# yewsiang/Transferable3D

Measured on AMD Instinct MI355X. Metric: frustums/sec fwd+bwd, higher is better.
Workload: dtype f32

## Files before the change

include/t3d.h:

```cpp
#ifndef T3D_H_
#define T3D_H_

#include <stdint.h>

#ifdef __cplusplus
extern "C" {
#endif

#define T3D_OK 0
#define T3D_ERR_ARG (-1)
#define T3D_ERR_SHAPE (-2)
#define T3D_ERR_LAUNCH (-3)
#define T3D_ERR_ABI (-4)

#define T3D_ABI_VERSION 3
#define T3D_V2_SIZE_pointmlp_fwd_args 200
#define T3D_V2_SIZE_pointmlp_dgrad_args 168
#define T3D_V2_SIZE_pointmlp_wgrad_args 144
#define T3D_V2_SIZE_pointmlp_dgrad_gram_args 168
#define T3D_V2_SIZE_pointmlp_gram_args 96
#define T3D_V2_SIZE_seg_head_args 208
#define T3D_V2_SIZE_boxpc_rep_args 104

#define T3D_TILE_ROWS 128
// ... 751 lines not shown
  const int32_t* choice;
  const int64_t* mask_offsets;
  uint64_t* masks;
  int32_t* seg_prefix;
  double* box2d_out;
  double* frustum_angle;
  int32_t* n_in_box;
  int32_t* count;
  int32_t* index;
  double* out_points;
  int32_t* label;
} t3d_frustum_extract_args;
#define T3D_V2_SIZE_frustum_extract_args 208
int t3d_frustum_extract(const t3d_frustum_extract_args* args, t3d_stream_t stream);

#ifdef __cplusplus
}
#endif
#endif
```

transferable3d_amd/abi.py:

```python
import ctypes as C
import os

F = C.POINTER(C.c_float)
I = C.POINTER(C.c_int32)
D = C.POINTER(C.c_double)
L = C.POINTER(C.c_int64)
i32, f32 = C.c_int, C.c_float

TILE_ROWS = 128
F32, BF16 = 0, 1
DTYPE_BY_NAME = {'f32': F32, 'bf16': BF16}
ARITH_AUTO, ARITH_FP32_MFMA, ARITH_BF16X3, ARITH_BF16 = 0, 1, 2, 3
ARITH_BY_NAME = {'auto': ARITH_AUTO, 'fp32_mfma': ARITH_FP32_MFMA, 'bf16x3': ARITH_BF16X3}
ARITH_NAMES = {ARITH_FP32_MFMA: 'fp32_mfma', ARITH_BF16X3: 'bf16x3', ARITH_BF16: 'bf16'}
ABI_VERSION = 3
ERR_ABI = -4
ACT_NONE, ACT_RELU, ACT_LEAKY_RELU, ACT_TANH = 0, 1, 2, 3
ACT_BY_NAME = {None: ACT_NONE, 'relu': ACT_RELU, 'leaky_relu': ACT_LEAKY_RELU, 'tanh': ACT_TANH}


class Sized(C.Structure):

    def __init__(self, *args, **kw):
        super().__init__(C.sizeof(type(self)), *args, **kw)
# ... 197 lines not shown
    _fields_ = [('off', C.c_int64), ('K', C.c_int32), ('N', C.c_int32), ('fwd', C.c_int32), ('dgrad', C.c_int32), ('blk0', C.c_int32), ('reserved', C.c_int32)]


def x3_frag_table(entries):
    import numpy as np
    rec = np.zeros(len(entries), dtype=np.dtype([('off', '<i8'), ('K', '<i4'), ('N', '<i4'), ('fwd', '<i4'), ('dgrad', '<i4'), ('blk0', '<i4'), ('reserved', '<i4')]))
    blk = 0
    for i, (off, K, N) in enumerate(entries):
        rec[i] = (off, K, N, 1, 1, blk, 0)
        blk += (K * N // 8 + 255) // 256
    return rec.view(np.uint8).copy(), blk


class SlabDesc(C.Structure):
    _fields_ = [('slab_off', C.c_int64), ('grad_off', C.c_int64), ('numel', C.c_int32), ('n_slabs', C.c_int32)]


class Schedule(C.Structure):
    _fields_ = [('base_lr', f32), ('lr_decay_rate', f32), ('lr_decay_step', f32), ('bn_init_decay', f32),
                ('bn_decay_rate', f32), ('bn_decay_step', f32), ('bn_decay_clip', f32), ('beta1', f32), ('beta2', f32),
                ('batch_size', i32), ('step_offset', i32)]


class BoxPcRepArgs(Sized):
    _fields_ = [('struct_size', C.c_uint32), ('pc', F), ('ld_pc', i32), ('C', i32), ('center', F), ('dims', F), ('theta', F), ('y_dims_cls', I),
                ('y_orient_cls', I), ('rep', F), ('ld_rep', i32), ('box_out', F), ('M', i32), ('rows_per_frustum', i32), ('rowmask', F)]


class BoxPcRepBArgs(C.Structure):
    _fields_ = [('center', F), ('dims', F), ('theta', F), ('y_dims_cls', I), ('y_orient_cls', I), ('box_out', F), ('pc', F), ('ld_pc', i32),
# ... 124 lines not shown
    't3d_boxpc_rep_b': [C.POINTER(BoxPcRepBArgs), VP],
    't3d_boxpc_rep_bwd': [C.POINTER(BoxPcRepBwdArgs), VP],
    't3d_boxpc_loss': [C.POINTER(BoxPcLossArgs), VP],
    't3d_pointmlp_dgrad_narrow': [C.POINTER(DgradNarrowArgs), VP],
    't3d_semi_final_loss': [C.POINTER(SemiFinalLossArgs), VP],
    't3d_anchor_reg_bwd': [C.POINTER(AnchorRegBwdArgs), VP],
    't3d_reduce_slabs': [F, F, C.POINTER(SlabDesc), i32, i32, VP],
    't3d_schedule_step': [F, C.POINTER(Schedule), VP],
    't3d_adam_tf_step': [F, F, F, F, C.c_int64, F, f32, f32, f32, f32, VP],
    't3d_momentum_step': [F, F, F, C.c_int64, F, f32, f32, VP],
    't3d_split_x3': [F, VP, C.c_int64, C.c_int64, VP],
    't3d_split_x3_frag': [F, VP, VP, C.c_int64, VP, i32, i32, VP],
    't3d_dropout_mask': [F, C.c_int64, f32, C.c_uint32, F, VP],
    't3d_cast_bf16': [F, VP, C.c_int64, VP],
    't3d_frustum_extract': [C.POINTER(FrustumExtractArgs), VP],
}

LIB_PATH = os.path.join(os.path.dirname(os.path.abspath(__file__)), 'libt3d.so')
ERRORS = {-1: 'T3D_ERR_ARG', -2: 'T3D_ERR_SHAPE', -3: 'T3D_ERR_LAUNCH'}


class T3DError(RuntimeError):
    pass


def source_hash_of(lib):
    buf = C.create_string_buffer(64)
    check(lib.t3d_source_hash(buf, 64), 't3d_source_hash')
    return buf.value.decode()

# ... 37 lines not shown
```

transferable3d_amd/csrc/bn_optim.hip:

```cpp
#include "common.h"
#include "poolbwd_dev.h"
#include "bn_dev.h"

namespace {

template <int GR, int CH = FC_CH>
__global__ __launch_bounds__(GR * CH) void k_bn_fwd_finalize(const t3d_bn_fwd_finalize_args p) {
  __shared__ double red[GR][CH];
  __shared__ float s_scsh[2 * CH];
  bn_fwd_finalize_body<GR, CH>(p, red, s_scsh, blockIdx.x);
}

__global__ __launch_bounds__(256) void k_pool_finalize(const t3d_pool_finalize_args p) {
  const int i = blockIdx.x * blockDim.x + threadIdx.x;
  if (i >= p.B * p.N) return;
  const int b = i / p.N, c = i % p.N;
  pool_pick_impl(p.pmax, p.pmin, p.pamax, p.pamin, p.tiles_per_frustum, p.N, b, c, p.scale[c], p.shift[c], p.pooled, p.ld_pooled,
                 p.argidx, p.ysel);
}

template <int GR, int CH = FC_CH>
__global__ __launch_bounds__(GR * CH) void k_bn_bwd_finalize(const t3d_bn_bwd_finalize_args p) {
  __shared__ double red[GR][CH];
  bn_bwd_finalize_body<GR, CH>(p, red, blockIdx.x, threadIdx.x);
// ... 53 lines not shown
    v[i] = vi;
    w[i] -= lr_t * mi / (sqrtf(vi) + eps);
  }
}

__global__ __launch_bounds__(256) void k_momentum_tf(float* __restrict__ w, const float* __restrict__ g, float* __restrict__ acc,
                                                     int64_t n, const float* __restrict__ hyper, float momentum, float gscale) {
  const float lr = hyper[1];
  for (int64_t i = (int64_t)blockIdx.x * blockDim.x + threadIdx.x; i < n; i += (int64_t)gridDim.x * blockDim.x) {
    const float a = fmaf(momentum, acc[i], g[i] * gscale);
    acc[i] = a;
    w[i] -= lr * a;
  }
}

__device__ __forceinline__ uint32_t mix_u32(uint64_t x) {
  x ^= x >> 33; x *= 0xff51afd7ed558ccdULL;
  x ^= x >> 33; x *= 0xc4ceb9fe1a85ec53ULL;
  x ^= x >> 33;
  return (uint32_t)(x >> 16);
}
__global__ __launch_bounds__(256) void k_dropout_mask(float* __restrict__ mask, int64_t n, float keep, uint32_t seed,
                                                      const float* __restrict__ hyper) {
  const uint64_t step = (uint64_t)hyper[0];
  const uint64_t key = ((uint64_t)seed << 32) ^ (step * 0x9E3779B97F4A7C15ULL);
  for (int64_t i = (int64_t)blockIdx.x * blockDim.x + threadIdx.x; i < n; i += (int64_t)gridDim.x * blockDim.x) {
    const uint32_t r = mix_u32(key + (uint64_t)i * 0xD6E8FEB86659FD93ULL);
    const float u = (float)(r >> 8) * (1.0f / 16777216.0f);
    mask[i] = u < keep ? 1.f : 0.f;
  }
// ... 87 lines not shown
  int64_t blocks = (n + 255) / 256;
  if (blocks > 2048) blocks = 2048;
  T3D_LAUNCH(k_adam_tf, dim3((unsigned)blocks), dim3(256), 0, static_cast<hipStream_t>(stream), params, grads, m,
                     v, n, hyper, beta1, beta2, eps, grad_scale);
  T3D_CHECK_LAUNCH();
  return T3D_OK;
}

extern "C" int t3d_momentum_step(float* params, const float* grads, float* accum, int64_t n, const float* hyper, float momentum,
                                 float grad_scale, t3d_stream_t stream) {
  if (!params || !grads || !accum || !hyper || n <= 0) return T3D_ERR_ARG;
  int64_t blocks = (n + 255) / 256;
  if (blocks > 2048) blocks = 2048;
  T3D_LAUNCH(k_momentum_tf, dim3((unsigned)blocks), dim3(256), 0, static_cast<hipStream_t>(stream), params, grads, accum, n, hyper,
             momentum, grad_scale);
  T3D_CHECK_LAUNCH();
  return T3D_OK;
}

__global__ __launch_bounds__(256) void k_cast_bf16(const float* __restrict__ src, bf16_t* __restrict__ dst, int64_t n) {
  const int64_t stride = (int64_t)gridDim.x * 256 * 8;
  for (int64_t i = ((int64_t)blockIdx.x * 256 + threadIdx.x) * 8; i < n; i += stride) {
    if (i + 8 <= n) {
      const float4 a = *reinterpret_cast<const float4*>(src + i), b = *reinterpret_cast<const float4*>(src + i + 4);
      const bf16x8 h = {(bf16_t)a.x, (bf16_t)a.y, (bf16_t)a.z, (bf16_t)a.w, (bf16_t)b.x, (bf16_t)b.y, (bf16_t)b.z, (bf16_t)b.w};
      *reinterpret_cast<bf16x8*>(dst + i) = h;
    } else {
      for (int64_t j = i; j < n; ++j) dst[j] = (bf16_t)src[j];
    }
  }
// ... 45 lines not shown
```

transferable3d_amd/csrc/common.h:

```cpp
#pragma once
#include <hip/hip_runtime.h>
#include <stdint.h>
#include "t3d.h"
#include "abi_take.h"

typedef float f32x16 __attribute__((ext_vector_type(16)));
typedef float f32x4 __attribute__((ext_vector_type(4)));

#define T3D_LAUNCH(...)          \
  do {                           \
    (void)hipGetLastError();     \
    hipLaunchKernelGGL(__VA_ARGS__); \
  } while (0)

#define T3D_CHECK_LAUNCH()                                  \
  do {                                                      \
    hipError_t e__ = hipGetLastError();                     \
    if (e__ != hipSuccess) return T3D_ERR_LAUNCH;           \
  } while (0)

__device__ __forceinline__ int xcd_remap(int bid, int nwg) {
  const int q = nwg >> 3, r = nwg & 7, xcd = bid & 7, idx = bid >> 3;
  const int base = (xcd < r) ? xcd * (q + 1) : r * (q + 1) + (xcd - r) * q;
  return base + idx;
// ... 39 lines not shown
  __device__ __forceinline__ static float ld1(const float* base, size_t i) { return (float)reinterpret_cast<const bf16_t*>(base)[i]; }
  __device__ __forceinline__ static void st1(float* base, size_t i, float v) { reinterpret_cast<bf16_t*>(base)[i] = (bf16_t)v; }
  __device__ __forceinline__ static void st2(float* base, size_t i, float a, float b) {
    bf16x2 v = {(bf16_t)a, (bf16_t)b};
    *reinterpret_cast<bf16x2*>(reinterpret_cast<bf16_t*>(base) + i) = v;
  }
  __device__ __forceinline__ static float rnd(float v) { return (float)(bf16_t)v; }
};

__device__ __forceinline__ float ld_elem(const float* base, size_t i, int dtype) {
  return dtype == T3D_BF16 ? Elem<bf16_t>::ld1(base, i) : base[i];
}
__device__ __forceinline__ float4 ld_elem4(const float* base, size_t i, int dtype) {
  return dtype == T3D_BF16 ? Elem<bf16_t>::widen(Elem<bf16_t>::ld4(base, i)) : *reinterpret_cast<const float4*>(base + i);
}
```

transferable3d_amd/csrc/pointmlp.hip:

```cpp
#include "common.h"
#include "poolbwd_dev.h"
#include "rider_dev.h"

#include <cstdlib>
#include <mutex>
#include <type_traits>
#include <utility>
#include <unordered_map>

namespace {

constexpr int BK = 32;
constexpr int MIN_WAVES_PER_EU = 2;
constexpr int LDR = BK + 4;
constexpr int NT = 256;

__device__ __forceinline__ float4 f4zero() { return make_float4(0.f, 0.f, 0.f, 0.f); }

__device__ __forceinline__ unsigned keep_bits32(const float* __restrict__ rowmask, int base) {
  float4 m[8];
#pragma unroll
  for (int q = 0; q < 8; ++q) m[q] = *reinterpret_cast<const float4*>(rowmask + base + (q >> 2) * 32 + (q & 3) * 8);
  unsigned bits = 0u;
#pragma unroll
// ... 665 lines not shown
    h_iter<1, TM, TN, SA, SB, LA, LB, AR, DIMA, BR, DIMB>(sa, sb, la, lb, smem, cur, last, last, a0, b0, acc, tid);
    cur ^= 1;
  }
  {
    const bf16_t* As = smem + cur * STAGE;
    const bf16_t* Bs = As + SA::LDS_ELEMS;
    mma_steps_h<TM, TN, AR, DIMA, BR, DIMB, 0, ST>(As, Bs, a0, b0, acc, tid & 63, [](int) {});
  }
  __syncthreads();
}

constexpr int BKX = 16;
constexpr int LDRX = BKX + 8;
constexpr int LDCX_PAD = 32;
__device__ __forceinline__ int x3_r_off(int row, int red) { return row * LDRX + red; }

__device__ __forceinline__ void split3(const float4& v, bf16x4& h, bf16x4& m, bf16x4& l) {
  const float x[4] = {v.x, v.y, v.z, v.w};
  unsigned hp[2], mp[2], lp[2];
  typedef float f32x2_ __attribute__((ext_vector_type(2)));
  auto pk = [](float a, float b) { const f32x2_ v = {a, b}; return __builtin_bit_cast(unsigned, __builtin_convertvector(v, bf16x2)); };
#pragma unroll
  for (int e = 0; e < 2; ++e) {
    const float x0 = x[2 * e], x1 = x[2 * e + 1];
    hp[e] = pk(x0, x1);
    float r0 = x0 - __uint_as_float(hp[e] << 16);
    asm("" : "+v"(r0));
    const float r1 = x1 - __uint_as_float(hp[e] & 0xffff0000u);
    mp[e] = pk(r0, r1);
    float s0 = r0 - __uint_as_float(mp[e] << 16);
    asm("" : "+v"(s0));
    const float s1 = r1 - __uint_as_float(mp[e] & 0xffff0000u);
    lp[e] = pk(s0, s1);
  }
  h = __builtin_bit_cast(bf16x4, make_uint2(hp[0], hp[1]));
  m = __builtin_bit_cast(bf16x4, make_uint2(mp[0], mp[1]));
  l = __builtin_bit_cast(bf16x4, make_uint2(lp[0], lp[1]));
}

struct WLoaderX3 {
  static constexpr bool PRESPLIT = true;
  const bf16_t* p;
  long stride;
  int ld;
  struct Raw { bf16x8 v; };
  struct Coef {};
  __device__ __forceinline__ Coef fetch_coef(int) const { return Coef(); }
  __device__ __forceinline__ Raw fetch(int plane, int row, int col) const {
    Raw r;
    r.v = *reinterpret_cast<const bf16x8*>(p + (size_t)plane * stride + (size_t)row * ld + col);
    return r;
  }
};
// ... 3725 lines not shown
```

transferable3d_amd/engine.py:

```python
import contextlib
import ctypes as C
import math
import os

import numpy as np
import torch

from . import abi
from .abi import fptr, iptr
from .constants import BN_EPS

TILE = abi.TILE_ROWS


class Runtime:

    def __init__(self, device=None, lib=None, gemm_arithmetic=None):
        self.lib = lib if lib is not None else abi.load()
        if gemm_arithmetic is None:
            gemm_arithmetic = 'fp32_mfma' if os.environ.get('T3D_X3', '1') == '0' else 'bf16x3'
        self.gemm_arithmetic = gemm_arithmetic
        self.arith = abi.ARITH_BY_NAME[gemm_arithmetic]
        if device is None:
            if not torch.cuda.is_available():
# ... 158 lines not shown
        n = int(np.prod(shape))
        n_pad = (n + 3) // 4 * 4
        if trainable:
            off = self.used
            assert off + n_pad <= self.params.numel(), 'VarStore capacity exceeded'
            self.used += n_pad
            buf = self.params
        else:
            off = self.state_used
            assert off + n_pad <= self.state.numel()
            self.state_used += n_pad
            buf = self.state
        self.index[name] = (off, tuple(shape), trainable)
        view = buf[off:off + n].view(*shape)
        view.copy_(torch.as_tensor(np.asarray(init, dtype=np.float32).reshape(shape)))
        return view

    def enable_bf16(self):
        if self.params16 is None:
            self.params16 = self.rt.zeros(self.params.numel(), dtype=torch.bfloat16)
        return self.params16

    def enable_x3(self):
        if getattr(self, 'params_x3', None) is None:
            self.params_x3 = self.rt.zeros(3 * self.params.numel(), dtype=torch.bfloat16)
        return self.params_x3

    def x3_ptr(self, w):
        off = (w.data_ptr() - self.params.data_ptr()) // 4
        if not (0 <= off and off + w.numel() <= self.params.numel() and w.is_contiguous()) or off % 4:
            return None, 0
        return self.enable_x3().data_ptr() + 2 * off, self.params.numel()

    def x3_frag(self, w, K, N):
        off = (w.data_ptr() - self.params.data_ptr()) // 4
        none = ((None, 0), (None, 0))
        if not (0 <= off and off + w.numel() <= self.params.numel() and w.is_contiguous()) or off % 8 or K % 32 or N % 32 or w.numel() != K * N:
            return none
        n = self.params.numel()
        stride = (n + 7) // 8 * 8
        if getattr(self, 'x3_frag_planes', None) is None:
            self.x3_frag_planes = (self.rt.zeros(3 * stride, dtype=torch.bfloat16), self.rt.zeros(3 * stride, dtype=torch.bfloat16))
            self.x3_frag_entries, self.x3_frag_stride, self.x3_frag_table = {}, stride, None
        self.x3_frag_entries[off] = (K, N)
        self.x3_frag_table = None
        pf, pd = self.x3_frag_planes
        return (pf.data_ptr() + 2 * off, stride), (pd.data_ptr() + 2 * off, stride)

    def frag_table(self):
        ent = getattr(self, 'x3_frag_entries', None)
        if not ent:
            return None
        if self.x3_frag_table is None:
            raw, blocks = abi.x3_frag_table([(off, K, N) for off, (K, N) in sorted(ent.items())])
            self.x3_frag_table = (torch.from_numpy(raw).to(self.rt.device), len(ent), blocks)
        return self.x3_frag_table

    def bf16_view(self, w):
        off = (w.data_ptr() - self.params.data_ptr()) // 4
        assert 0 <= off and off + w.numel() <= self.params.numel() and w.is_contiguous()
        return self.enable_bf16()[off:off + w.numel()].view(*w.shape)

    def get(self, name):
        off, shape, trainable = self.index[name]
        buf = self.params if trainable else self.state
        return buf[off:off + int(np.prod(shape))].view(*shape)

    def grad(self, name):
        off, shape, trainable = self.index[name]
        assert trainable
        return self.grads[off:off + int(np.prod(shape))].view(*shape)
# ... 11 lines not shown
        return self._alloc(name, shape, trainable, np.full(shape, val, np.float32))

    def state_dict(self):
        return {k: self.get(k).detach().cpu().numpy().copy() for k in self.index}

    def load_state_dict(self, sd, strict=True):
        for k, v in sd.items():
            if k not in self.index:
                if strict:
                    raise KeyError(k)
                continue
            v = np.asarray(v, dtype=np.float32)
            if v.size != int(np.prod(self.index[k][1])):
                raise ValueError('variable %s: the state holds shape %s, the graph declares %s' % (k, v.shape, self.index[k][1]))
            self.get(k).copy_(torch.as_tensor(v).reshape(self.index[k][1]))

    def trainable_ranges(self, prefixes=None):
        items = sorted((off, int(np.prod(shape)), name) for name, (off, shape, tr) in self.index.items() if tr)
        out = []
        for off, n, name in items:
            if prefixes is not None and not any(name.startswith(p) for p in prefixes):
                continue
            n_pad = (n + 3) // 4 * 4
            if out and out[-1][0] + out[-1][1] == off:
                out[-1][1] += n_pad
            else:
                out.append([off, n_pad])
        return [(o, n) for o, n in out]


# ... 542 lines not shown
```

transferable3d_amd/nets.py:

```python
import ctypes as C
import os

import numpy as np
import torch

from . import abi
from .abi import fptr, iptr
from .constants import BOX_OUT_DIMS, NUM_CLASS
from .engine import ActSpec, FcLayer, Plan, PointLayer, Runtime, VarStore, Workspace, TILE


class Graph:

    def __init__(self, batch_size, num_point, num_channel, rt=None, seed=0, unbiased_ema=True, vars=None, dtype='f32'):
        assert dtype in ('f32', 'bf16')
        self.dtype = dtype
        self.dt = abi.DTYPE_BY_NAME[dtype]
        self.adt = torch.bfloat16 if dtype == 'bf16' else torch.float32
        if num_point % TILE:
            raise abi.T3DError('num_point must be a multiple of %d' % TILE)
        self.rt = rt or Runtime()
        self.B, self.rpf, self.C = batch_size, num_point, num_channel
        self.ldpc = (num_channel + 3) // 4 * 4
        self.M = batch_size * num_point
# ... 25 lines not shown
        return self

    def emit_reduce_slabs(self, plan):
        ws, vs, lib = self.ws, self.vars, self.rt.lib
        plan.join()
        i0, i1 = self._slabs_reduced, len(ws.entries)
        self._slabs_reduced = i1
        if i1 == i0:
            return
        mx = max(e[2] for e in ws.entries[i0:i1])
        stride = C.sizeof(abi.SlabDesc)

        def thunk(s):
            return lib.t3d_reduce_slabs(fptr(ws.buf), fptr(vs.grads),
                                        C.cast(C.c_void_p(ws.table.data_ptr() + i0 * stride), C.POINTER(abi.SlabDesc)), i1 - i0, mx, s)
        plan.add_raw('t3d_reduce_slabs', thunk)

    def emit_cast_weights(self, plan):
        vs, lib = self.vars, self.rt.lib
        if self.dt != abi.BF16:
            from .engine import X3_PRESPLIT
            if (X3_PRESPLIT and self.rt.device.type == 'cuda' and self.rt.arith != abi.ARITH_FP32_MFMA and getattr(vs, 'x3_frag_enabled', True)
                    and hasattr(lib, 't3d_split_x3_frag')):
                def thunk(s):
                    if not getattr(vs, 'x3_frag_entries', None):
                        return 0
                    t, n, nblk = vs.frag_table()
                    pf, pd = vs.x3_frag_planes
                    return lib.t3d_split_x3_frag(fptr(vs.params), C.c_void_p(pf.data_ptr()), C.c_void_p(pd.data_ptr()), vs.x3_frag_stride,
                                                 C.c_void_p(t.data_ptr()), n, nblk, s)
                plan.add_raw('t3d_split_x3_frag', thunk)
            return
        p16 = vs.enable_bf16()
        plan.add_raw('t3d_cast_bf16', lambda s: lib.t3d_cast_bf16(fptr(vs.params), C.c_void_p(p16.data_ptr()), vs.used, s))

    def default_bucket(self):
        return self.vars.trainable_ranges(self.trained_prefixes)

    def declare_bucket(self, plan, prefixes):
        if not self.dp_buckets:
            return
        self.emit_reduce_slabs(plan)
        self.buckets.append(self.vars.trainable_ranges(prefixes))
        plan.bucket_ready(len(self.buckets) - 1)

# ... 22 lines not shown
        lib, hyper = self.rt.lib, self.hyper
        plan.add_raw('t3d_schedule_step', lambda s: lib.t3d_schedule_step(fptr(hyper), C.byref(sched), s), sched)

    def emit_dropout_masks(self, plan, seed=1234):
        lib, hyper = self.rt.lib, self.hyper
        for i, (scope, (mask, keep)) in enumerate(sorted(self.dropout_masks.items())):
            plan.add_raw('t3d_dropout_mask',
                         lambda s, mask=mask, keep=keep, sd=seed + 7919 * i: lib.t3d_dropout_mask(
                             fptr(mask), mask.numel(), keep, sd, fptr(hyper), s))

    def emit_adam(self, plan, prefixes=None, beta1=0.9, beta2=0.999, eps=1e-8, grad_scale=1.0):
        lib, vs, hyper = self.rt.lib, self.vars, self.hyper
        vs.optimizer_kind = 'adam'

        def adam(off, n):
            plan.add_raw('t3d_adam_tf_step',
                         lambda s, off=off, n=n: lib.t3d_adam_tf_step(
                             fptr(vs.params[off:]), fptr(vs.grads[off:]), fptr(vs.adam_m[off:]), fptr(vs.adam_v[off:]),
                             n, fptr(hyper), beta1, beta2, eps, grad_scale, s))
        self._emit_optimizer(plan, prefixes, adam)

    def emit_momentum(self, plan, prefixes=None, momentum=0.9, grad_scale=1.0):
        lib, vs, hyper = self.rt.lib, self.vars, self.hyper
        vs.optimizer_kind = 'momentum'

        def mom(off, n):
            plan.add_raw('t3d_momentum_step',
                         lambda s, off=off, n=n: lib.t3d_momentum_step(
                             fptr(vs.params[off:]), fptr(vs.grads[off:]), fptr(vs.adam_m[off:]), n, fptr(hyper), momentum, grad_scale, s))
        self._emit_optimizer(plan, prefixes, mom)

    def _emit_optimizer(self, plan, prefixes, launch):
        vs = self.vars
        self.trained_prefixes = prefixes
        ranges = vs.trainable_ranges(prefixes)
        if self.buckets:
            covered = sorted(r for b in self.buckets for r in b)
            assert sum(n for _, n in covered) == sum(n for _, n in ranges) and \
                all(any(o >= ro and o + n <= ro + rn for ro, rn in ranges) for o, n in covered), \
                'gradient buckets must partition the trained variables'
            for i, b in enumerate(self.buckets):
                plan.bucket_wait(i)
                for off, n in b:
                    launch(off, n)
# ... 971 lines not shown
```

transferable3d_amd/step.py:

```python
import os

import torch

from . import abi
from .engine import Plan


OPTIMIZER_CALLS = ('t3d_adam_tf_step', 't3d_momentum_step')


class TrainStep:
    def __init__(self, engine, pre, fwd, bwd=None, opt=None, process_group=None, use_hip_graph=None, force_dist=False,
                 one_graph=None):
        self.e, self.rt = engine, engine.rt
        self.pre, self.fwd, self.bwd, self.opt = pre, fwd, bwd, opt
        self.train = bwd is not None
        self.pg = process_group
        self.world = process_group.size() if process_group is not None else 1
        self.dist = self.train and process_group is not None and (self.world > 1 or force_dist)
        self.on_gpu = self.rt.device.type == 'cuda'
        want = use_hip_graph if use_hip_graph is not None else self.on_gpu
        self.want_graph = bool(want) and self.on_gpu
        env = os.environ.get('T3D_DP_ONE_GRAPH', '')
        if one_graph is None:
# ... 30 lines not shown
            for (name, call, arg), lane in zip(p.calls, p.lanes):
                if name == 't3d_dropout_mask' and not generate_masks:
                    continue
                calls.append((name, call, arg))
                lanes.append(lane)
            calls.append((Plan.JOIN, lambda s: 0, None))
            lanes.append(0)
            two = two or p.two_streams
        if self.dist and not any(c[0] == Plan.BUCKET for c in calls):
            k = next((i for i, c in enumerate(calls) if c[0] in OPTIMIZER_CALLS), len(calls))
            calls[k:k] = [(Plan.BUCKET, lambda s: 0, 0), (Plan.WAIT, lambda s: 0, 0)]
            lanes[k:k] = [0, 0]
        if not two:
            calls, lanes = self._overlap(calls, lanes)
            two = two or getattr(self, 'two_stream', False)
        prog, cur = [], Plan(self.rt)
        cur.two_streams = two

        def close():
            nonlocal cur
            if len(cur):
                prog.append(('run', cur))
            cur = Plan(self.rt)
            cur.two_streams = two

        for (name, call, arg), lane in zip(calls, lanes):
            if name in (Plan.BUCKET, Plan.WAIT):
                if self.dist:
                    close()
                    prog.append(('allreduce' if name == Plan.BUCKET else 'wait', arg))
# ... 32 lines not shown
        S_calls, T_calls = real(calls[sb:se]), real(calls[tb:sb])
        if self._two_stream_overlap(S_calls + T_calls):
            self.two_stream = True
            first, second = (T_calls, S_calls) if os.environ.get('T3D_TWO_STREAM_FIRST', 'S') == 'T' else (S_calls, T_calls)
            lanes2 = [0] * tb + [1] * len(first) + [0] + [0] * len(second) + [0]
            merged = first + [(Plan.FLUSH, lambda s: 0, None)] + second + [(Plan.JOIN, lambda s: 0, None)]
            calls = calls[:tb] + merged + calls[se + 1:]
            lanes2 += [0] * (len(calls) - len(lanes2))
            self.schedule_report = {'mode': 'two streams', 'S_launches': len(S_calls), 'T_launches': len(T_calls), 'hosted': 0, 'rider_ops': 0,
                                    'pairs': 0, 'solo': len(S_calls) + len(T_calls)}
            return calls, lanes2
        if self._sets is None:
            self._sets = schedule.RiderSets(self.rt)
        merged, self.schedule_report = schedule.overlap_chains(self.rt, S_calls, T_calls, self._sets)
        return calls[:tb] + merged + calls[se + 1:], lanes[:tb] + [0] * len(merged) + lanes[se + 1:]

    def _two_stream_overlap(self, chain_calls):
        mode = os.environ.get('T3D_OVERLAP_STREAMS', '')
        if mode in ('0', '1'):
            return mode == '1' and self.on_gpu
        if not self.on_gpu:
            return False
        return self.e.M >= 4 * 32768

    def _shares_gpu(self):
        if not self.on_gpu or os.environ.get('T3D_RIDERS_SHARED_GPU', '0') == '1':
            return False
        local_ranks = int(os.environ.get('LOCAL_WORLD_SIZE', self.world))
        return local_ranks > torch.cuda.device_count()

# ... 88 lines not shown
                graphs[k] = g
        return prog, graphs

    def run(self, generate_masks=True):
        self.n_runs += 1
        self._issue(generate_masks)
        if self._sets is not None and self.rider_check_every > 0 and self.n_runs % self.rider_check_every == 0:
            self.check_riders()

    def _issue(self, generate_masks):
        key = bool(generate_masks)
        ent = self.cache.get(key)
        if ent is None:
            ent = self.cache[key] = {'prog': self._program(key), 'graphs': None, 'runs': 0}
        ent['runs'] += 1
        if not self.want_graph or ent['runs'] == 1:
            return self._run_program(ent['prog'])
        if ent['graphs'] is None:
            prog, graphs = self._capture(ent['prog'])
            ent['cprog'], ent['graphs'] = prog, graphs
            if self._sets is not None:
                self._sets.timeouts()
        if ent['cprog'] and ent['cprog'][0][0] == 'run_graph':
            ent['graphs'][0].replay()
            return
        self._run_program(ent['cprog'], ent['graphs'])

    def dp_report(self):
        mode = 'flat' if len(self._buckets()) == 1 else 'bucketed'
        if self.one_graph:
# ... 211 lines not shown
```

Measured before the change: 27290.

## Fuse slab reduction, optimizer update and x3 weight split into one kernel

Adds a fused optimizer kernel driven by a per-block descriptor table. In one launch it sums gradient slabs, applies the Adam or momentum update, and writes the bf16x3 split weight planes for fragment tiles. The step program drops the separate reduce_slabs and split_x3_frag launches, which removes extra passes over params and grads and a few kernel launches per step. The cost is tracking when the planes are valid on the host, a tile layout that writes the planes from small 8x32 tiles, and a fallback to the old path whenever the setup does not fit the fused layout.

```diff
diff --git a/include/t3d.h b/include/t3d.h
--- a/include/t3d.h
+++ b/include/t3d.h
@@ -789,6 +789,39 @@
 #define T3D_V2_SIZE_frustum_extract_args 208
 int t3d_frustum_extract(const t3d_frustum_extract_args* args, t3d_stream_t stream);
 
+enum { T3D_OPT_FLAT = 0, T3D_OPT_SLAB = 1, T3D_OPT_TILE = 2 };
+enum { T3D_OPT_ADAM = 0, T3D_OPT_MOMENTUM = 1 };
+typedef struct {
+  int32_t kind;
+  int32_t count;
+  int64_t start;
+  int64_t slab_off;
+  int32_t n_slabs;
+  int32_t numel;
+  int64_t off;
+  int32_t K, N;
+  int32_t k0, n0;
+  int32_t fwd, dgrad;
+} t3d_opt_block;
+typedef struct {
+  uint32_t struct_size;
+  int32_t kind;
+  float* params;
+  float* grads;
+  float* m;
+  float* v;
+  const float* slab_base;
+  void* planes_fwd;
+  void* planes_dgrad;
+  int64_t plane_stride;
+  const t3d_opt_block* blocks;
+  int32_t n_blocks;
+  const float* hyper;
+  float beta1, beta2, eps, momentum, grad_scale;
+} t3d_optimizer_fused_args;
+#define T3D_V2_SIZE_optimizer_fused_args 120
+int t3d_optimizer_fused(const t3d_optimizer_fused_args* args, t3d_stream_t stream);
+
 #ifdef __cplusplus
 }
 #endif
diff --git a/transferable3d_amd/abi.py b/transferable3d_amd/abi.py
--- a/transferable3d_amd/abi.py
+++ b/transferable3d_amd/abi.py
@@ -235,6 +235,55 @@
 
 class SlabDesc(C.Structure):
     _fields_ = [('slab_off', C.c_int64), ('grad_off', C.c_int64), ('numel', C.c_int32), ('n_slabs', C.c_int32)]
+
+
+OPT_FLAT, OPT_SLAB, OPT_TILE = 0, 1, 2
+OPT_ADAM, OPT_MOMENTUM = 0, 1
+OPT_FLAT_ELEMS, OPT_SLAB_ELEMS = 1024, 256
+
+
+class OptimizerFusedArgs(Sized):
+    _fields_ = [('struct_size', C.c_uint32), ('kind', C.c_int32), ('params', C.c_void_p), ('grads', C.c_void_p), ('m', C.c_void_p), ('v', C.c_void_p),
+                ('slab_base', C.c_void_p), ('planes_fwd', C.c_void_p), ('planes_dgrad', C.c_void_p), ('plane_stride', C.c_int64),
+                ('blocks', C.c_void_p), ('n_blocks', C.c_int32), ('hyper', C.c_void_p), ('beta1', C.c_float), ('beta2', C.c_float),
+                ('eps', C.c_float), ('momentum', C.c_float), ('grad_scale', C.c_float)]
+
+
+def optimizer_fused_blocks(off, n, slabs, frags):
+    import numpy as np
+    dt = np.dtype([('kind', '<i4'), ('count', '<i4'), ('start', '<i8'), ('slab_off', '<i8'), ('n_slabs', '<i4'), ('numel', '<i4'), ('off', '<i8'),
+                   ('K', '<i4'), ('N', '<i4'), ('k0', '<i4'), ('n0', '<i4'), ('fwd', '<i4'), ('dgrad', '<i4')])
+    assert dt.itemsize == 64
+    end = off + n
+    by_off = {}
+    for so, go, ne, ns in slabs:
+        if go < off or go + ne > end or ne <= 0 or ns <= 0 or go in by_off:
+            return None
+        by_off[go] = (so, ne, ns)
+    recs, covered = [], []
+    for fo, K, N, fwd, dgrad in frags:
+        if fo < off or fo + K * N > end or fo % 8 or K % 32 or N % 32:
+            return None
+        so, ne, ns = by_off.pop(fo, (0, K * N, 0))
+        if ne != K * N or so % 4:
+            return None
+        covered.append((fo, K * N))
+        for k0 in range(0, K, 8):
+            for n0 in range(0, N, 32):
+                recs.append((OPT_TILE, 0, 0, so, ns, ne, fo, K, N, k0, n0, int(bool(fwd)), int(bool(dgrad))))
+    for go, (so, ne, ns) in sorted(by_off.items()):
+        covered.append((go, ne))
+        for s0 in range(0, ne, OPT_SLAB_ELEMS):
+            recs.append((OPT_SLAB, min(OPT_SLAB_ELEMS, ne - s0), go + s0, so, ns, ne, go, 0, 0, 0, 0, 0, 0))
+    pos = off
+    for co, cn in sorted(covered) + [(end, 0)]:
+        if co < pos:
+            return None
+        for s0 in range(pos, co, OPT_FLAT_ELEMS):
+            recs.append((OPT_FLAT, min(OPT_FLAT_ELEMS, co - s0), s0, 0, 0, 0, 0, 0, 0, 0, 0, 0, 0))
+        pos = co + cn
+    recs.sort(key=lambda r: -(r[4] if r[0] != OPT_FLAT else 0))
+    return np.array(recs, dtype=dt)
 
 
 class Schedule(C.Structure):
@@ -389,6 +438,7 @@
     't3d_dropout_mask': [F, C.c_int64, f32, C.c_uint32, F, VP],
     't3d_cast_bf16': [F, VP, C.c_int64, VP],
     't3d_frustum_extract': [C.POINTER(FrustumExtractArgs), VP],
+    't3d_optimizer_fused': [C.POINTER(OptimizerFusedArgs), VP],
 }
 
 LIB_PATH = os.path.join(os.path.dirname(os.path.abspath(__file__)), 'libt3d.so')
diff --git a/transferable3d_amd/csrc/bn_optim.hip b/transferable3d_amd/csrc/bn_optim.hip
--- a/transferable3d_amd/csrc/bn_optim.hip
+++ b/transferable3d_amd/csrc/bn_optim.hip
@@ -91,6 +91,170 @@
   }
 }
 
+__device__ __forceinline__ float opt_elem(const t3d_optimizer_fused_args& p, const bool adam, const float lr_t, const float lr, const float w,
+                                          const float g, float& m, float& v) {
+#pragma clang fp contract(off)
+  if (adam) {
+    const float gi = g * p.grad_scale;
+    const float mi = p.beta1 * m + (1.f - p.beta1) * gi;
+    const float vi = p.beta2 * v + (1.f - p.beta2) * gi * gi;
+    m = mi;
+    v = vi;
+    return w - lr_t * mi / (sqrtf(vi) + p.eps);
+  }
+  const float a = fmaf(p.momentum, m, g * p.grad_scale);
+  m = a;
+  return fmaf(-lr, a, w);
+}
+
+__device__ __forceinline__ float4 opt_elem4(const t3d_optimizer_fused_args& p, const bool adam, const float lr_t, const float lr, const float4 w,
+                                            const float4 g, float4& m, float4& v) {
+  float4 r;
+  r.x = opt_elem(p, adam, lr_t, lr, w.x, g.x, m.x, v.x);
+  r.y = opt_elem(p, adam, lr_t, lr, w.y, g.y, m.y, v.y);
+  r.z = opt_elem(p, adam, lr_t, lr, w.z, g.z, m.z, v.z);
+  r.w = opt_elem(p, adam, lr_t, lr, w.w, g.w, m.w, v.w);
+  return r;
+}
+
+__device__ __forceinline__ float4 slab_group_sum(const float4* __restrict__ s, const size_t n4, const int n_slabs, const int grp) {
+  float4 a0 = make_float4(0.f, 0.f, 0.f, 0.f), a1 = a0, a2 = a0, a3 = a0;
+  int k = grp;
+  for (; k + 56 < n_slabs; k += 64) {
+    float4 v[8];
+#pragma unroll
+    for (int u = 0; u < 8; ++u) v[u] = s[(size_t)(k + 8 * u) * n4];
+#pragma unroll
+    for (int u = 0; u < 8; u += 4) {
+      a0.x += v[u].x; a0.y += v[u].y; a0.z += v[u].z; a0.w += v[u].w;
+      a1.x += v[u + 1].x; a1.y += v[u + 1].y; a1.z += v[u + 1].z; a1.w += v[u + 1].w;
+      a2.x += v[u + 2].x; a2.y += v[u + 2].y; a2.z += v[u + 2].z; a2.w += v[u + 2].w;
+      a3.x += v[u + 3].x; a3.y += v[u + 3].y; a3.z += v[u + 3].z; a3.w += v[u + 3].w;
+    }
+  }
+  for (; k + 24 < n_slabs; k += 32) {
+    const float4 v0 = s[(size_t)(k + 0) * n4], v1 = s[(size_t)(k + 8) * n4], v2 = s[(size_t)(k + 16) * n4], v3 = s[(size_t)(k + 24) * n4];
+    a0.x += v0.x; a0.y += v0.y; a0.z += v0.z; a0.w += v0.w;
+    a1.x += v1.x; a1.y += v1.y; a1.z += v1.z; a1.w += v1.w;
+    a2.x += v2.x; a2.y += v2.y; a2.z += v2.z; a2.w += v2.w;
+    a3.x += v3.x; a3.y += v3.y; a3.z += v3.z; a3.w += v3.w;
+  }
+  for (; k < n_slabs; k += 8) {
+    const float4 v = s[(size_t)k * n4];
+    a0.x += v.x; a0.y += v.y; a0.z += v.z; a0.w += v.w;
+  }
+  float4 r;
+  r.x = (a0.x + a1.x) + (a2.x + a3.x); r.y = (a0.y + a1.y) + (a2.y + a3.y);
+  r.z = (a0.z + a1.z) + (a2.z + a3.z); r.w = (a0.w + a1.w) + (a2.w + a3.w);
+  return r;
+}
+
+constexpr int OPT_FLAT_ELEMS = 1024;
+constexpr int OPT_SLAB_ELEMS = 256;
+
+__global__ __launch_bounds__(512) void k_optimizer_fused(const t3d_optimizer_fused_args p) {
+  __shared__ float4 part[8][64];
+  __shared__ float wt[8][33];
+  const t3d_opt_block bl = p.blocks[blockIdx.x];
+  const int tid = threadIdx.x;
+  const bool adam = p.kind == T3D_OPT_ADAM;
+  const float lr_t = p.hyper[3], lr = p.hyper[1];
+  float4 zero = make_float4(0.f, 0.f, 0.f, 0.f);
+  if (bl.kind == T3D_OPT_FLAT) {
+    const int rem = bl.count - 4 * tid;
+    if (tid >= OPT_FLAT_ELEMS / 4 || rem <= 0) return;
+    const int64_t i = bl.start + 4 * tid;
+    if (rem >= 4 && (i & 3) == 0) {
+      float4 m = *reinterpret_cast<const float4*>(p.m + i), v = adam ? *reinterpret_cast<const float4*>(p.v + i) : zero;
+      const float4 w = opt_elem4(p, adam, lr_t, lr, *reinterpret_cast<const float4*>(p.params + i), *reinterpret_cast<const float4*>(p.grads + i), m, v);
+      *reinterpret_cast<float4*>(p.m + i) = m;
+      if (adam) *reinterpret_cast<float4*>(p.v + i) = v;
+      *reinterpret_cast<float4*>(p.params + i) = w;
+    } else {
+      for (int64_t j = i; j < i + (rem < 4 ? rem : 4); ++j) {
+        float m = p.m[j], v = adam ? p.v[j] : 0.f;
+        p.params[j] = opt_elem(p, adam, lr_t, lr, p.params[j], p.grads[j], m, v);
+        p.m[j] = m;
+        if (adam) p.v[j] = v;
+      }
+    }
+    return;
+  }
+  const bool tile = bl.kind == T3D_OPT_TILE;
+  if (!tile && ((bl.slab_off | bl.off | (int64_t)bl.numel) & 3) != 0) {
+    if (tid >= bl.count) return;
+    const int64_t e = bl.start - bl.off + tid, j = bl.start + tid;
+    float acc = 0.f;
+    for (int k = 0; k < bl.n_slabs; ++k) acc += p.slab_base[bl.slab_off + (size_t)k * bl.numel + e];
+    p.grads[j] = acc;
+    float m = p.m[j], v = adam ? p.v[j] : 0.f;
+    p.params[j] = opt_elem(p, adam, lr_t, lr, p.params[j], acc, m, v);
+    p.m[j] = m;
+    if (adam) p.v[j] = v;
+    return;
+  }
+  const int el = tid & 63, grp = tid >> 6;
+  const size_t n4 = (size_t)(bl.numel >> 2);
+  const size_t e4 = tile ? (((size_t)(bl.k0 + (el >> 3)) * bl.N + bl.n0) >> 2) + (el & 7) : (size_t)((bl.start - bl.off) >> 2) + el;
+  const bool live = el < (tile ? 64 : (bl.count >> 2));
+  const bool upd = grp == 0 && live;
+  const size_t ue = (size_t)(bl.off >> 2) + e4;
+  float4 w4 = zero, m4 = zero, v4 = zero, g4 = zero;
+  if (upd) {
+    w4 = reinterpret_cast<const float4*>(p.params)[ue];
+    m4 = reinterpret_cast<const float4*>(p.m)[ue];
+    if (adam) v4 = reinterpret_cast<const float4*>(p.v)[ue];
+    if (bl.n_slabs <= 0) g4 = reinterpret_cast<const float4*>(p.grads)[ue];
+  }
+  if (bl.n_slabs > 0) {
+    part[grp][el] = live ? slab_group_sum(reinterpret_cast<const float4*>(p.slab_base + bl.slab_off) + e4, n4, bl.n_slabs, grp) : zero;
+    __syncthreads();
+    if (upd) {
+      g4 = part[0][el];
+#pragma unroll
+      for (int g = 1; g < 8; ++g) {
+        const float4 u = part[g][el];
+        g4.x += u.x; g4.y += u.y; g4.z += u.z; g4.w += u.w;
+      }
+      reinterpret_cast<float4*>(p.grads)[ue] = g4;
+    }
+  }
+  if (upd) {
+    w4 = opt_elem4(p, adam, lr_t, lr, w4, g4, m4, v4);
+    reinterpret_cast<float4*>(p.m)[ue] = m4;
+    if (adam) reinterpret_cast<float4*>(p.v)[ue] = v4;
+    reinterpret_cast<float4*>(p.params)[ue] = w4;
+    if (tile) {
+      float* d = &wt[tid >> 3][(tid & 7) * 4];
+      d[0] = w4.x; d[1] = w4.y; d[2] = w4.z; d[3] = w4.w;
+    }
+  }
+  if (!tile) return;
+  __syncthreads();
+  bf16x4 h0, m0, l0, h1, m1, l1;
+  if (tid < 32 && bl.fwd) {
+    const int NB = bl.N / 32;
+    const long f = ((long)(bl.k0 >> 4) * NB + (bl.n0 >> 5)) * 64 + (((bl.k0 >> 3) & 1) << 5) + tid;
+    split3(make_float4(wt[0][tid], wt[1][tid], wt[2][tid], wt[3][tid]), h0, m0, l0);
+    split3(make_float4(wt[4][tid], wt[5][tid], wt[6][tid], wt[7][tid]), h1, m1, l1);
+    bf16_t* d = static_cast<bf16_t*>(p.planes_fwd) + bl.off + f * 8;
+    *reinterpret_cast<bf16x8*>(d) = __builtin_shufflevector(h0, h1, 0, 1, 2, 3, 4, 5, 6, 7);
+    *reinterpret_cast<bf16x8*>(d + p.plane_stride) = __builtin_shufflevector(m0, m1, 0, 1, 2, 3, 4, 5, 6, 7);
+    *reinterpret_cast<bf16x8*>(d + 2 * p.plane_stride) = __builtin_shufflevector(l0, l1, 0, 1, 2, 3, 4, 5, 6, 7);
+  }
+  if (tid >= 64 && tid < 96 && bl.dgrad) {
+    const int t = tid - 64, r = t >> 2, k = bl.k0 + r, nn = bl.n0 + 8 * (t & 3), KB = bl.K / 32;
+    const long f = ((long)(nn >> 4) * KB + (k >> 5)) * 64 + (((nn >> 3) & 1) << 5) + (k & 31);
+    const float* src = &wt[r][8 * (t & 3)];
+    split3(make_float4(src[0], src[1], src[2], src[3]), h0, m0, l0);
+    split3(make_float4(src[4], src[5], src[6], src[7]), h1, m1, l1);
+    bf16_t* d = static_cast<bf16_t*>(p.planes_dgrad) + bl.off + f * 8;
+    *reinterpret_cast<bf16x8*>(d) = __builtin_shufflevector(h0, h1, 0, 1, 2, 3, 4, 5, 6, 7);
+    *reinterpret_cast<bf16x8*>(d + p.plane_stride) = __builtin_shufflevector(m0, m1, 0, 1, 2, 3, 4, 5, 6, 7);
+    *reinterpret_cast<bf16x8*>(d + 2 * p.plane_stride) = __builtin_shufflevector(l0, l1, 0, 1, 2, 3, 4, 5, 6, 7);
+  }
+}
+
 __device__ __forceinline__ uint32_t mix_u32(uint64_t x) {
   x ^= x >> 33; x *= 0xff51afd7ed558ccdULL;
   x ^= x >> 33; x *= 0xc4ceb9fe1a85ec53ULL;
@@ -208,6 +372,23 @@
   if (blocks > 2048) blocks = 2048;
   T3D_LAUNCH(k_momentum_tf, dim3((unsigned)blocks), dim3(256), 0, static_cast<hipStream_t>(stream), params, grads, accum, n, hyper,
              momentum, grad_scale);
+  T3D_CHECK_LAUNCH();
+  return T3D_OK;
+}
+
+static_assert(sizeof(t3d_optimizer_fused_args) == T3D_V2_SIZE_optimizer_fused_args && sizeof(t3d_opt_block) == 64, "t3d.h: t3d_optimizer_fused");
+
+extern "C" int t3d_optimizer_fused(const t3d_optimizer_fused_args* a, t3d_stream_t stream) {
+  T3D_ABI_TAKE(optimizer_fused_args, a);
+  if (!a || !a->params || !a->grads || !a->m || !a->hyper || !a->blocks || a->n_blocks <= 0) return T3D_ERR_ARG;
+  if (a->kind != T3D_OPT_ADAM && a->kind != T3D_OPT_MOMENTUM) return T3D_ERR_ARG;
+  if (a->kind == T3D_OPT_ADAM && !a->v) return T3D_ERR_ARG;
+  auto misaligned = [](const void* q) { return (reinterpret_cast<uintptr_t>(q) & 15) != 0; };
+  if (misaligned(a->params) || misaligned(a->grads) || misaligned(a->m) || misaligned(a->v) || misaligned(a->slab_base) ||
+      misaligned(a->planes_fwd) || misaligned(a->planes_dgrad) || (reinterpret_cast<uintptr_t>(a->blocks) & 7))
+    return T3D_ERR_ARG;
+  if ((a->planes_fwd || a->planes_dgrad) && (a->plane_stride <= 0 || (a->plane_stride & 7))) return T3D_ERR_ARG;
+  T3D_LAUNCH(k_optimizer_fused, dim3((unsigned)a->n_blocks), dim3(512), 0, static_cast<hipStream_t>(stream), *a);
   T3D_CHECK_LAUNCH();
   return T3D_OK;
 }
diff --git a/transferable3d_amd/csrc/common.h b/transferable3d_amd/csrc/common.h
--- a/transferable3d_amd/csrc/common.h
+++ b/transferable3d_amd/csrc/common.h
@@ -77,3 +77,26 @@
 __device__ __forceinline__ float4 ld_elem4(const float* base, size_t i, int dtype) {
   return dtype == T3D_BF16 ? Elem<bf16_t>::widen(Elem<bf16_t>::ld4(base, i)) : *reinterpret_cast<const float4*>(base + i);
 }
+
+__device__ __forceinline__ void split3(const float4& v, bf16x4& h, bf16x4& m, bf16x4& l) {
+  const float x[4] = {v.x, v.y, v.z, v.w};
+  unsigned hp[2], mp[2], lp[2];
+  typedef float f32x2_ __attribute__((ext_vector_type(2)));
+  auto pk = [](float a, float b) { const f32x2_ v = {a, b}; return __builtin_bit_cast(unsigned, __builtin_convertvector(v, bf16x2)); };
+#pragma unroll
+  for (int e = 0; e < 2; ++e) {
+    const float x0 = x[2 * e], x1 = x[2 * e + 1];
+    hp[e] = pk(x0, x1);
+    float r0 = x0 - __uint_as_float(hp[e] << 16);
+    asm("" : "+v"(r0));
+    const float r1 = x1 - __uint_as_float(hp[e] & 0xffff0000u);
+    mp[e] = pk(r0, r1);
+    float s0 = r0 - __uint_as_float(mp[e] << 16);
+    asm("" : "+v"(s0));
+    const float s1 = r1 - __uint_as_float(mp[e] & 0xffff0000u);
+    lp[e] = pk(s0, s1);
+  }
+  h = __builtin_bit_cast(bf16x4, make_uint2(hp[0], hp[1]));
+  m = __builtin_bit_cast(bf16x4, make_uint2(mp[0], mp[1]));
+  l = __builtin_bit_cast(bf16x4, make_uint2(lp[0], lp[1]));
+}
diff --git a/transferable3d_amd/csrc/pointmlp.hip b/transferable3d_amd/csrc/pointmlp.hip
--- a/transferable3d_amd/csrc/pointmlp.hip
+++ b/transferable3d_amd/csrc/pointmlp.hip
@@ -703,29 +703,6 @@
 constexpr int LDRX = BKX + 8;
 constexpr int LDCX_PAD = 32;
 __device__ __forceinline__ int x3_r_off(int row, int red) { return row * LDRX + red; }
-
-__device__ __forceinline__ void split3(const float4& v, bf16x4& h, bf16x4& m, bf16x4& l) {
-  const float x[4] = {v.x, v.y, v.z, v.w};
-  unsigned hp[2], mp[2], lp[2];
-  typedef float f32x2_ __attribute__((ext_vector_type(2)));
-  auto pk = [](float a, float b) { const f32x2_ v = {a, b}; return __builtin_bit_cast(unsigned, __builtin_convertvector(v, bf16x2)); };
-#pragma unroll
-  for (int e = 0; e < 2; ++e) {
-    const float x0 = x[2 * e], x1 = x[2 * e + 1];
-    hp[e] = pk(x0, x1);
-    float r0 = x0 - __uint_as_float(hp[e] << 16);
-    asm("" : "+v"(r0));
-    const float r1 = x1 - __uint_as_float(hp[e] & 0xffff0000u);
-    mp[e] = pk(r0, r1);
-    float s0 = r0 - __uint_as_float(mp[e] << 16);
-    asm("" : "+v"(s0));
-    const float s1 = r1 - __uint_as_float(mp[e] & 0xffff0000u);
-    lp[e] = pk(s0, s1);
-  }
-  h = __builtin_bit_cast(bf16x4, make_uint2(hp[0], hp[1]));
-  m = __builtin_bit_cast(bf16x4, make_uint2(mp[0], mp[1]));
-  l = __builtin_bit_cast(bf16x4, make_uint2(lp[0], lp[1]));
-}
 
 struct WLoaderX3 {
   static constexpr bool PRESPLIT = true;
diff --git a/transferable3d_amd/engine.py b/transferable3d_amd/engine.py
--- a/transferable3d_amd/engine.py
+++ b/transferable3d_amd/engine.py
@@ -196,6 +196,8 @@
         self.index[name] = (off, tuple(shape), trainable)
         view = buf[off:off + n].view(*shape)
         view.copy_(torch.as_tensor(np.asarray(init, dtype=np.float32).reshape(shape)))
+        if trainable:
+            self.invalidate_planes()
         return view
 
     def enable_bf16(self):
@@ -224,8 +226,11 @@
         if getattr(self, 'x3_frag_planes', None) is None:
             self.x3_frag_planes = (self.rt.zeros(3 * stride, dtype=torch.bfloat16), self.rt.zeros(3 * stride, dtype=torch.bfloat16))
             self.x3_frag_entries, self.x3_frag_stride, self.x3_frag_table = {}, stride, None
-        self.x3_frag_entries[off] = (K, N)
-        self.x3_frag_table = None
+            self.x3_frag_tables_kept = []
+        if self.x3_frag_entries.get(off) != (K, N):
+            self.x3_frag_entries[off] = (K, N)
+            self.x3_frag_table = None
+            self.invalidate_planes()
         pf, pd = self.x3_frag_planes
         return (pf.data_ptr() + 2 * off, stride), (pd.data_ptr() + 2 * off, stride)
 
@@ -236,7 +241,31 @@
         if self.x3_frag_table is None:
             raw, blocks = abi.x3_frag_table([(off, K, N) for off, (K, N) in sorted(ent.items())])
             self.x3_frag_table = (torch.from_numpy(raw).to(self.rt.device), len(ent), blocks)
+            self.x3_frag_tables_kept.append(self.x3_frag_table[0])
         return self.x3_frag_table
+
+    def invalidate_planes(self):
+        self.x3_planes_epoch = getattr(self, 'x3_planes_epoch', 0) + 1
+
+    def _planes_state(self):
+        return (self.params._version, getattr(self, 'x3_planes_epoch', 0))
+
+    def planes_valid(self):
+        return getattr(self, 'x3_planes_mark', None) == self._planes_state()
+
+    def mark_planes_valid(self):
+        self.x3_planes_mark = self._planes_state()
+
+    def refresh_planes(self, stream=None):
+        if self.planes_valid() or not getattr(self, 'x3_frag_entries', None):
+            return False
+        t, n, nblk = self.frag_table()
+        pf, pd = self.x3_frag_planes
+        abi.check(self.rt.lib.t3d_split_x3_frag(abi.fptr(self.params), C.c_void_p(pf.data_ptr()), C.c_void_p(pd.data_ptr()), self.x3_frag_stride,
+                                                C.c_void_p(t.data_ptr()), n, nblk, stream if stream is not None else self.rt.stream()),
+                  't3d_split_x3_frag')
+        self.mark_planes_valid()
+        return True
 
     def bf16_view(self, w):
         off = (w.data_ptr() - self.params.data_ptr()) // 4
@@ -278,6 +307,7 @@
             if v.size != int(np.prod(self.index[k][1])):
                 raise ValueError('variable %s: the state holds shape %s, the graph declares %s' % (k, v.shape, self.index[k][1]))
             self.get(k).copy_(torch.as_tensor(v).reshape(self.index[k][1]))
+        self.invalidate_planes()
 
     def trainable_ranges(self, prefixes=None):
         items = sorted((off, int(np.prod(shape)), name) for name, (off, shape, tr) in self.index.items() if tr)
diff --git a/transferable3d_amd/nets.py b/transferable3d_amd/nets.py
--- a/transferable3d_amd/nets.py
+++ b/transferable3d_amd/nets.py
@@ -63,6 +63,7 @@
         def thunk(s):
             return lib.t3d_reduce_slabs(fptr(ws.buf), fptr(vs.grads),
                                         C.cast(C.c_void_p(ws.table.data_ptr() + i0 * stride), C.POINTER(abi.SlabDesc)), i1 - i0, mx, s)
+        thunk.fuse = {'op': 'reduce', 'entries': (i0, i1)}
         plan.add_raw('t3d_reduce_slabs', thunk)
 
     def emit_cast_weights(self, plan):
@@ -78,6 +79,7 @@
                     pf, pd = vs.x3_frag_planes
                     return lib.t3d_split_x3_frag(fptr(vs.params), C.c_void_p(pf.data_ptr()), C.c_void_p(pd.data_ptr()), vs.x3_frag_stride,
                                                  C.c_void_p(t.data_ptr()), n, nblk, s)
+                thunk.fuse = {'op': 'split'}
                 plan.add_raw('t3d_split_x3_frag', thunk)
             return
         p16 = vs.enable_bf16()
@@ -130,10 +132,12 @@
         vs.optimizer_kind = 'adam'
 
         def adam(off, n):
-            plan.add_raw('t3d_adam_tf_step',
-                         lambda s, off=off, n=n: lib.t3d_adam_tf_step(
-                             fptr(vs.params[off:]), fptr(vs.grads[off:]), fptr(vs.adam_m[off:]), fptr(vs.adam_v[off:]),
-                             n, fptr(hyper), beta1, beta2, eps, grad_scale, s))
+            def thunk(s):
+                vs.invalidate_planes()
+                return lib.t3d_adam_tf_step(fptr(vs.params[off:]), fptr(vs.grads[off:]), fptr(vs.adam_m[off:]), fptr(vs.adam_v[off:]),
+                                            n, fptr(hyper), beta1, beta2, eps, grad_scale, s)
+            thunk.fuse = {'op': 'adam', 'range': (off, n), 'beta1': beta1, 'beta2': beta2, 'eps': eps, 'momentum': 0.0, 'grad_scale': grad_scale}
+            plan.add_raw('t3d_adam_tf_step', thunk)
         self._emit_optimizer(plan, prefixes, adam)
 
     def emit_momentum(self, plan, prefixes=None, momentum=0.9, grad_scale=1.0):
@@ -141,9 +145,11 @@
         vs.optimizer_kind = 'momentum'
 
         def mom(off, n):
-            plan.add_raw('t3d_momentum_step',
-                         lambda s, off=off, n=n: lib.t3d_momentum_step(
-                             fptr(vs.params[off:]), fptr(vs.grads[off:]), fptr(vs.adam_m[off:]), n, fptr(hyper), momentum, grad_scale, s))
+            def thunk(s):
+                vs.invalidate_planes()
+                return lib.t3d_momentum_step(fptr(vs.params[off:]), fptr(vs.grads[off:]), fptr(vs.adam_m[off:]), n, fptr(hyper), momentum, grad_scale, s)
+            thunk.fuse = {'op': 'momentum', 'range': (off, n), 'beta1': 0.0, 'beta2': 0.0, 'eps': 0.0, 'momentum': momentum, 'grad_scale': grad_scale}
+            plan.add_raw('t3d_momentum_step', thunk)
         self._emit_optimizer(plan, prefixes, mom)
 
     def _emit_optimizer(self, plan, prefixes, launch):
diff --git a/transferable3d_amd/step.py b/transferable3d_amd/step.py
--- a/transferable3d_amd/step.py
+++ b/transferable3d_amd/step.py
@@ -6,7 +6,7 @@
 from .engine import Plan
 
 
-OPTIMIZER_CALLS = ('t3d_adam_tf_step', 't3d_momentum_step')
+OPTIMIZER_CALLS = ('t3d_adam_tf_step', 't3d_momentum_step', 't3d_optimizer_fused')
 
 
 class TrainStep:
@@ -68,6 +68,7 @@
         if not two:
             calls, lanes = self._overlap(calls, lanes)
             two = two or getattr(self, 'two_stream', False)
+        calls, lanes = self._fuse_tail(calls, lanes)
         prog, cur = [], Plan(self.rt)
         cur.two_streams = two
 
@@ -130,6 +131,60 @@
             self._sets = schedule.RiderSets(self.rt)
         merged, self.schedule_report = schedule.overlap_chains(self.rt, S_calls, T_calls, self._sets)
         return calls[:tb] + merged + calls[se + 1:], lanes[:tb] + [0] * len(merged) + lanes[se + 1:]
+
+    def _fuse_tail(self, calls, lanes):
+        import ctypes as C
+        import numpy as np
+        e, vs, lib = self.e, self.e.vars, self.rt.lib
+        self.planes_on_demand = self.fused_tail = False
+        tag = lambda c: getattr(c[1], 'fuse', None) or {}
+        real = lambda c: not c[0].startswith('__')
+        splits = [i for i, c in enumerate(calls) if c[0] == 't3d_split_x3_frag' and tag(c).get('op') == 'split']
+        if not (self.on_gpu and splits and getattr(vs, 'x3_frag_entries', None)):
+            return calls, lanes
+        drop, put = set(splits), {}
+        if self.train:
+            opts = [i for i, c in enumerate(calls) if c[0] in OPTIMIZER_CALLS]
+            if self.dist or not hasattr(lib, 't3d_optimizer_fused') or not opts or getattr(e.ws, 'buf', None) is None:
+                return calls, lanes
+            if any(tag(calls[i]).get('op') not in ('adam', 'momentum') for i in opts) or \
+                    any(real(c) and i not in opts for i, c in enumerate(calls) if i > opts[0]):
+                return calls, lanes
+            j = opts[0] - 1
+            while j >= 0 and not real(calls[j]):
+                j -= 1
+            slabs = []
+            if j >= 0 and calls[j][0] == 't3d_reduce_slabs' and tag(calls[j]).get('op') == 'reduce':
+                i0, i1 = tag(calls[j])['entries']
+                slabs = list(e.ws.entries[i0:i1])
+                drop.add(j)
+            frags = sorted((off, K, N) for off, (K, N) in vs.x3_frag_entries.items())
+            hyper, (pf, pd) = e.hyper, vs.x3_frag_planes
+            for i in opts:
+                t = tag(calls[i])
+                off, n = t['range']
+                mine = [x for x in slabs if off <= x[1] < off + n]
+                slabs = [x for x in slabs if x not in mine]
+                blocks = abi.optimizer_fused_blocks(off, n, mine, [(fo, K, N, 1, 1) for fo, K, N in frags if off <= fo < off + n])
+                if blocks is None:
+                    return calls, lanes
+                dev = torch.from_numpy(blocks.view(np.uint8).copy()).to(self.rt.device)
+                a = abi.OptimizerFusedArgs(
+                    abi.OPT_ADAM if t['op'] == 'adam' else abi.OPT_MOMENTUM, vs.params.data_ptr(), vs.grads.data_ptr(), vs.adam_m.data_ptr(),
+                    vs.adam_v.data_ptr(), e.ws.buf.data_ptr(), pf.data_ptr(), pd.data_ptr(), vs.x3_frag_stride, dev.data_ptr(), len(blocks),
+                    hyper.data_ptr(), t['beta1'], t['beta2'], t['eps'], t['momentum'], t['grad_scale'])
+                put[i] = ('t3d_optimizer_fused', lambda s, a=a, keep=(dev, hyper, pf, pd): lib.t3d_optimizer_fused(C.byref(a), s), None)
+            if slabs:
+                host = (abi.SlabDesc * len(slabs))(*[abi.SlabDesc(*x) for x in slabs])
+                tab = torch.from_numpy(np.frombuffer(bytes(host), dtype=np.uint8).copy()).to(self.rt.device)
+                mx, ws, ns = max(x[2] for x in slabs), e.ws, len(slabs)
+                put[j] = ('t3d_reduce_slabs', lambda s, tab=tab: lib.t3d_reduce_slabs(
+                    abi.fptr(ws.buf), abi.fptr(vs.grads), C.cast(C.c_void_p(tab.data_ptr()), C.POINTER(abi.SlabDesc)), ns, mx, s), None)
+                drop.discard(j)
+            self.fused_tail = True
+        self.planes_on_demand = True
+        out = [(put.get(i, c), l) for i, (c, l) in enumerate(zip(calls, lanes)) if i not in drop]
+        return [c for c, _ in out], [l for _, l in out]
 
     def _two_stream_overlap(self, chain_calls):
         mode = os.environ.get('T3D_OVERLAP_STREAMS', '')
@@ -248,6 +303,21 @@
         if ent is None:
             ent = self.cache[key] = {'prog': self._program(key), 'graphs': None, 'runs': 0}
         ent['runs'] += 1
+        vs = self.e.vars
+        if getattr(self, 'planes_on_demand', False):
+            vs.refresh_planes()
+        try:
+            self._issue_program(ent)
+        except BaseException:
+            vs.invalidate_planes()
+            raise
+        if self.train:
+            if getattr(self, 'fused_tail', False):
+                vs.mark_planes_valid()
+            else:
+                vs.invalidate_planes()
+
+    def _issue_program(self, ent):
         if not self.want_graph or ent['runs'] == 1:
             return self._run_program(ent['prog'])
         if ent['graphs'] is None:
```

Result: no change. 27500 (median of 6 runs) (+0.8%).
